# jopohl/urh

Hardware: AMD Instinct MI355X
Metric: Msamples/s IQ->bits (1 GiB complex64 2-FSK per GPU, qad materialised, compact outputs copied to the host) (higher is better)
Workload: dtype f32

## Files before the change

include/urhgpu.h:

```cpp
#ifndef URHGPU_H
#define URHGPU_H

#include <stdint.h>

#ifdef __cplusplus
extern "C" {
#endif

#define URHGPU_VERSION 100

#define URHGPU_OK 0
#define URHGPU_ERR_HIP (-1)
#define URHGPU_ERR_DTYPE (-2)
#define URHGPU_ERR_ARG (-3)
#define URHGPU_ERR_CAPACITY (-4)
#define URHGPU_ERR_UNSUPPORTED (-5)
#define URHGPU_ERR_NO_DEVICE (-6)

#define URHGPU_DT_I8 0
#define URHGPU_DT_U8 1
#define URHGPU_DT_I16 2
#define URHGPU_DT_U16 3
#define URHGPU_DT_F32 4

// ... 268 lines not shown
int urhgpu_test_hot_probe(urhgpu_ctx *ctx, const void *d_iq, int64_t n, const urhgpu_params *p, float *d_qad, int stream_kind, int event_mode,
                          int graded, int launches, int keep, void *d_chunks_out, int64_t *n_chunks_out, float *dur_ms, float *gap_ms, int bubble_us,
                          int load_kind);
int urhgpu_test_hot_stamps(int on);
int urhgpu_test_tail_skip(int mask);
int urhgpu_test_fetch_chunk_tables(urhgpu_ctx *ctx, void *host_dst, int64_t n_chunks);
int urhgpu_memcpy_to_host(urhgpu_ctx *ctx, const void *d_src, void *host_dst, int64_t bytes);
int urhgpu_memcpy_dtod(urhgpu_ctx *ctx, void *d_dst, const void *d_src, int64_t bytes);

int urhgpu_test_force_state_bytes(int on);

int urhgpu_test_force_generic_tail(int on);

int urhgpu_test_force_tiles_per_chunk(int tiles);

int64_t urhgpu_test_wide_int_launches(void);

int64_t urhgpu_test_costas_host_syncs(void);
int64_t urhgpu_test_center_host_syncs(void);
int urhgpu_test_costas_scratch(int64_t n, int loop_order, int64_t *out3);

int urhgpu_test_atan2f_dev(urhgpu_ctx *ctx, const float *d_y, const float *d_x, int64_t n, float *d_out);

int urhgpu_chunk_power_stats_dev(urhgpu_ctx *ctx, const void *d_src, int dtype, int64_t n_rows, void *d_dst, int64_t n_store, double *sum_out,
                                 double *max_out);
int urhgpu_chunk_stats_launches(urhgpu_ctx *ctx, int64_t *n_launches);

int urhgpu_magnitude_chunk_partials_dev(urhgpu_ctx *ctx, const void *d_iq, int dtype, int64_t n_local, int64_t pos_base, int64_t n_total,
                                        int64_t chunk, int64_t n_chunks, double *d_sum, double *d_max);
#define URHGPU_PW_REC_HEAD 8
// ... 63 lines not shown
```

urh_amd/_lib.py:

```python
import ctypes as C
import os
import threading

HERE = os.path.dirname(os.path.abspath(__file__))
LIB_PATH = os.path.join(HERE, "liburhgpu.so")

OK = 0
ERR_HIP, ERR_DTYPE, ERR_ARG, ERR_CAPACITY, ERR_UNSUPPORTED, ERR_NO_DEVICE = -1, -2, -3, -4, -5, -6
BLOB_LEN16 = 2
BLOB_ROW16 = 4

DT_I8, DT_U8, DT_I16, DT_U16, DT_F32 = 0, 1, 2, 3, 4
MOD_ASK, MOD_FSK, MOD_PSK, MOD_OTHER = 0, 1, 2, 3
ROW_ABSORBED = -(1 << 62)
BLOB_MAGIC = 0x55524842424C4F42
BLOB_HEADER_BYTES = 128


class UrhGpuError(RuntimeError):
    def __init__(self, status, msg):
        super().__init__(msg)
        self.status = status


# ... 161 lines not shown
    "urhgpu_modulate_gfsk": (_i, [_vp, _vp, _i64, C.c_uint32, _vp, _i, _f, _f, _f, C.c_uint32, C.c_uint32, _i, _vp, _i, _vp, _vp]),
    "urhgpu_spectrogram_dev": (_i, [_vp, _vp, _i64, _i, _i64, _i64, _vp, _vp, _vp, _vp]),
    "urhgpu_bgra_lookup_dev": (_i, [_vp, _vp, _i64, _i, _vp, _i, _f, _f, _vp]),
    "urhgpu_convert_dev": (_i, [_vp, _vp, _i, _vp, _i, _i64]),
    "urhgpu_pcm_to_iq_dev": (_i, [_vp, _vp, _i64, _i, _i, _vp]),
    "urhgpu_sub_encode_runs": (_i, [_vp, _i64, _i64, _vp, _i64, _vp]),
    "urhgpu_fft_peak_dev": (_i, [_vp, _vp, _i64, _vp]),
    "urhgpu_astype_dev": (_i, [_vp, _vp, _i, _vp, _i, _i64]),
    "urhgpu_path_minmax_dev": (_i, [_vp, _vp, _i, _i64, _i64, _i64, _vp]),
    "urhgpu_path_minmax": (_i, [_vp, _vp, _i, _i64, _i64, _i64, _i64, _vp]),
    "urhgpu_bench_copy_ceiling_dev": (_i, [_vp, _vp, _vp, _i64, _i, _i, C.POINTER(_f)]),
    "urhgpu_memcpy_to_host": (_i, [_vp, _vp, _vp, _i64]),
    "urhgpu_memcpy_dtod": (_i, [_vp, _vp, _vp, _i64]),
    "urhgpu_test_force_state_bytes": (_i, [_i]),
    "urhgpu_test_force_tiles_per_chunk": (_i, [_i]),
    "urhgpu_test_wide_int_launches": (_i64, []),
    "urhgpu_test_costas_host_syncs": (_i64, []),
    "urhgpu_test_costas_scratch": (_i, [_i64, _i, C.POINTER(_i64)]),
    "urhgpu_test_force_generic_tail": (_i, [_i]),
    "urhgpu_test_atan2f_dev": (_i, [_vp, _vp, _vp, _i64, _vp]),
    "urhgpu_chunk_power_stats_dev": (_i, [_vp, _vp, _i, _i64, _vp, _i64, C.POINTER(C.c_double), C.POINTER(C.c_double)]),
    "urhgpu_chunk_stats_launches": (_i, [_vp, C.POINTER(_i64)]),
    "urhgpu_magnitude_chunk_partials_dev": (_i, [_vp, _vp, _i, _i64, _i64, _i64, _i64, _i64, _vp, _vp]),
    "urhgpu_pairwise_partial_f32_dev": (_i, [_vp, _vp, _i64, _i64, _i64, _i, _f, _vp, _i64, C.POINTER(_i64)]),
    "urhgpu_dc_correct_dev": (_i, [_vp, _vp, _i64, _i, _vp, _vp]),
    "urhgpu_dc_correct": (_i, [_vp, _vp, _i64, _i, _vp, _vp]),
    "urhgpu_test_dc_host_syncs": (_i64, []),
    "urhgpu_test_dc_stats": (_i, [_vp, C.POINTER(_i64)]),
    "urhgpu_shard_dc_sums_dev": (_i, [_vp, _vp, _i64, _i, _vp]),
    "urhgpu_shard_dc_spec_dev": (_i, [_vp, _vp, _i64, C.POINTER(C.c_double), _vp]),
# ... 158 lines not shown
```

urh_amd/csrc/launchers.hpp:

```cpp
#pragma once
#include <atomic>
#include <hip/hip_runtime.h>
#include <stdint.h>

#include "common.hpp"
#include "runs.hpp"

namespace urh {

struct RunArgs {
    const void *in;
    float *qad;
    const void *left_halo;
    int64_t n;
    int64_t range_begin;
    int64_t range_end;
    int64_t chunk_base;
    int64_t pos_base;
    int64_t chunk_len;
    uint64_t *slab;
    int64_t slab_stride;
    ChunkInfo *chunks;
    float noise_sqrd;
    float noise_val;
// ... 7 lines not shown
    uint32_t *progress;
    int32_t n_seg;
    int32_t seg_end[kMaxSegments];
    int64_t launch_lo, launch_hi;
    int64_t graded_from, graded_len;
    int wide_int;
    int stamp_probe;
    float thr[kMaxOrder - 1];
    const float *d_thr;
    const float *d_noise;
};
extern bool g_force_state_bytes;
extern std::atomic<long long> g_wide_int_launches;
extern bool g_stamp_probe;
extern int g_tail_skip;
struct HotEvents { hipEvent_t start = nullptr, stop = nullptr; bool used = false; };
int launch_wide_probe(const void *d_iq, int dtype, int64_t n, float noise_sqrd, int32_t *h_out, hipStream_t s, const float *d_noise = nullptr);
int launch_demod_runs_iq(const RunArgs &a, int dtype, int mod, bool write_qad, hipStream_t s, HotEvents *ev = nullptr);
int launch_runs_qad(const RunArgs &a, hipStream_t s, HotEvents *ev = nullptr);
bool runs_streamable(const RunArgs &a);
int launch_afp_demod(const RunArgs &a, int dtype, int mod, int grid, hipStream_t s);
int launch_afp_seam(const RunArgs &a, int dtype, int mod, float *d_out, hipStream_t s);
void launch_test_div(uint64_t seed, int reps, unsigned long long *d_mismatches, hipStream_t s);
void launch_test_sincosf_fast(unsigned long long *d_mismatches, hipStream_t s);
void launch_test_atan2f(const float *y, const float *x, int64_t n, float *out, hipStream_t s);

struct ModMsg {
    int64_t bit_off;
    int64_t n_sym;
    int64_t sym_off;
// ... 285 lines not shown
```

urh_amd/csrc/probes.hip:

```cpp
#include "pass.hpp"

using namespace urh;

#define URH_PROBE_WPB 4

namespace urh {
bool g_tile_tail = true;
int g_force_tiles_per_chunk = 0;
}

extern "C" {

int urhgpu_test_fast_division_dev(urhgpu_ctx *ctx, uint64_t seed, int reps, uint64_t *n_mismatch) {
    if (!ctx || !n_mismatch || reps < 0) return URHGPU_ERR_ARG;
    URH_HIP(hipSetDevice(ctx->device));
    URH_HIP(hipMemsetAsync(ctx->d_counts, 0, 8, ctx->stream));
    launch_test_div(seed, reps, (unsigned long long *)ctx->d_counts, ctx->stream);
    URH_HIP(hipGetLastError());
    URH_TRY(fetch_out(ctx, ctx->h_counts, ctx->d_counts, 8));
    *n_mismatch = (uint64_t)ctx->h_counts[0];
    return URHGPU_OK;
}

int urhgpu_test_force_merge_ambiguous(int on) {
// ... 156 lines not shown
int urhgpu_test_force_generic_tail(int on) { urh::g_tile_tail = (on == 0); return URHGPU_OK; }
int64_t urhgpu_test_wide_int_launches(void) { return (int64_t)urh::g_wide_int_launches.load(); }
int64_t urhgpu_test_costas_host_syncs(void) { return (int64_t)urh::g_costas_host_syncs.load(); }
int urhgpu_test_costas_scratch(int64_t n, int loop_order, int64_t *out3) {
    if (!out3 || n < 0 || (loop_order != 2 && loop_order != 4)) return URHGPU_ERR_ARG;
    urh::costas_scratch_layout(n, loop_order == 4 ? 8 : 4, out3);
    return URHGPU_OK;
}

int urhgpu_test_force_tiles_per_chunk(int tiles) {
    if (tiles < 0 || tiles > 4) return URHGPU_ERR_ARG;
    urh::g_force_tiles_per_chunk = tiles;
    return URHGPU_OK;
}

int urhgpu_test_atan2f_dev(urhgpu_ctx *ctx, const float *d_y, const float *d_x, int64_t n, float *d_out) {
    if (!ctx) return URHGPU_ERR_ARG;
    URH_HIP(hipSetDevice(ctx->device));
    launch_test_atan2f(d_y, d_x, n, d_out, ctx->stream);
    URH_HIP(hipGetLastError());
    return URHGPU_OK;
}

}
```

urh_amd/csrc/pulse_table.hip:

```cpp
#include <hip/hip_runtime.h>

#include <algorithm>

#include "common.hpp"
#include "compact.hpp"
#include "launchers.hpp"
#include "runs.hpp"
#include "scan.hpp"

namespace urh {

#ifndef URH_RESOLVE_BLOCK
#define URH_RESOLVE_BLOCK 256
#endif
#ifndef URH_RESOLVE_ITEMS
#define URH_RESOLVE_ITEMS 4
#endif
constexpr int kResolveBlock = URH_RESOLVE_BLOCK;

__host__ __device__ static inline int64_t resolve_blocks(int64_t n_chunks) { return (n_chunks + kResolveBlock - 1) / kResolveBlock; }

size_t resolve_scratch_bytes(int64_t n_chunks) {
    return (size_t)n_chunks * (4 * 4 + 2 * 8) + (size_t)(resolve_blocks(n_chunks) + 1) * (4 + 4 + 8) + 10 * 256;
}
// ... 624 lines not shown
}
__device__ __forceinline__ ResElem res_of_chunk(int cnt, uint32_t c_first_state, uint32_t c_last_state, uint32_t c_pend_state, int64_t c_last_pos,
                                                int64_t c_pend_pos, int pend_stable) {
    const bool pend_in = pend_stable && (cnt == 0 || c_pend_state != c_last_state);
    const int k = cnt + (pend_in ? 1 : 0);
    if (k == 0) return res_identity();
    const uint32_t first_state = cnt > 0 ? c_first_state : c_pend_state;
    const int64_t last_pos = pend_in ? c_pend_pos : c_last_pos;
    const uint32_t last_state = pend_in ? c_pend_state : c_last_state;
    return res_make(first_state, k == 1 ? last_pos : -1, last_state, k - 1, k >= 2, last_pos, last_state);
}

struct TileTail {
    ResElem *ploc;
    ResElem *btot;
    VecK<4> *agg;
    VecK<4> *excl;
    int64_t *tile_off;
    int32_t *tile_cnt;
    int64_t *d_n_tiles;
    int32_t *huge_count;
    int parity;
    int want_bits;
    GranDesc *rdesc;
    unsigned long long epoch;
    int64_t *d_row_base;
    int64_t *esc;
};

__global__ __launch_bounds__(kResolveBlock) void k_resolve_one(const ResolveArgs a, const TileTail ft, const int64_t blk0, const SegGate gate) {
// ... 46 lines not shown
    if (lane == 63) s_w[wave] = incl;
    __syncthreads();
    ResElem base = res_identity(), tot = res_identity();
#pragma unroll
    for (int w = 0; w < kResolveBlock / 64; ++w) {
        if (w < wave) base = res_combine(base, s_w[w]);
        tot = res_combine(tot, s_w[w]);
    }
    ResElem ex = res_shfl_up(incl, 1);
    if (lane == 0) ex = res_identity();
    ex = res_combine(base, ex);
    if (c < a.n_chunks) ft.ploc[c] = ex;
    if (t == 0) ft.btot[blk] = tot;
}

__device__ __forceinline__ ResElem res_fold_blocks(const ResElem *btot, int64_t count, int lane, ResElem first) {
    ResElem carry = res_identity();
    for (int64_t u0 = 0; u0 < count; u0 += 64) {
        ResElem x = first;
        if (u0 > 0) { x = res_identity(); if (u0 + lane < count) x = btot[u0 + lane]; }
        x = res_wave_incl_scan(x, lane);
        carry = res_combine(carry, res_shfl(x, 63));
    }
    return carry;
}

__device__ __forceinline__ ResElem res_before_entry(const TileTail &ft, const ResElem &init, int64_t c, int64_t n_chunks, int lane) {
    const int64_t nb = (c >= n_chunks) ? resolve_blocks(n_chunks) : c / kResolveBlock;
    ResElem first = res_identity();
    if (lane < nb) first = ft.btot[lane];
    ResElem pre = res_combine(init, res_fold_blocks(ft.btot, nb, lane, first));
    if (c < n_chunks) pre = res_combine(pre, ft.ploc[c]);
    return pre;
}

struct ShardPart { ResElem tot; int32_t first_nonlead, open_chunk; };
__global__ __launch_bounds__(kResolveBlock) void k_shard_summary(const ResolveArgs a, ShardPart *part, int32_t *ticket) {
    URH_TAIL_PRIO();
    __shared__ ResElem s_w[kResolveBlock / 64];
    __shared__ int32_t s_fn[kResolveBlock / 64], s_oc[kResolveBlock / 64];
    __shared__ bool s_last;
    const int64_t c = (int64_t)blockIdx.x * kResolveBlock + threadIdx.x;
    const int t = threadIdx.x, lane = t & 63, wave = t >> 6;
    ResElem e = res_identity();
    int32_t fn = kAuxNone, oc = kAuxNone;
    if (c < a.n_chunks) {
        const ChunkInfo *ch = a.chunks + c;
        const int64_t pend_pos = ch->pend_pos, start = ch->start, len = ch->len, last_pos = ch->last_pos, own_lead = ch->lead;
// ... 125 lines not shown
#else
#define URH_EMIT_OCC
#endif
#ifdef URH_OCC_EXPAND
#define URH_EXPAND_OCC __attribute__((amdgpu_waves_per_eu(URH_OCC_EXPAND)))
#else
#define URH_EXPAND_OCC URH_TAIL_OCC
#endif
static_assert(kResolveBlock % kTailCPW == 0 && kTailCPW <= 64, "the chunks of one wavefront share their resolve workgroup");

__device__ __forceinline__ int64_t lane_bcast(int64_t v, int src) {
    const int lo = __builtin_amdgcn_readlane((int)(uint32_t)(uint64_t)v, src), hi = __builtin_amdgcn_readlane((int)(uint32_t)((uint64_t)v >> 32), src);
    return (int64_t)(((uint64_t)(uint32_t)hi << 32) | (uint32_t)lo);
}
__device__ __forceinline__ int lane_bcast(int v, int src) { return __builtin_amdgcn_readlane(v, src); }

struct EmitTileArgs {
    EmitArgs e;
    ResolveArgs r;
    TileTail ft;
    BitsParams bp;
    HugeRef *huge;
    int32_t huge_cap;
    int64_t w0, w_end;
    int final_seg;
    SegState *seg;
    int seg_k;
    int8_t *h_state;
    int32_t *h_len;
    int len16;
// ... 12 lines not shown
            const unsigned long long slot = atomicAdd((unsigned long long *)g.esc, 1ull);
            if ((int64_t)slot < g.esc_cap) g.esc[1 + slot] = (int64_t)(((uint64_t)(uint32_t)(int32_t)len << 32) | (uint64_t)(uint32_t)idx);
        }
        return;
    }
    g.h_state[idx] = (int8_t)state;
    if (!g.len16) { g.h_len[idx] = (int32_t)len; return; }
    const bool fits = len >= 0 && len < 0xFFFF;
    ((uint16_t *)g.h_len)[idx] = fits ? (uint16_t)len : (uint16_t)0xFFFF;
    if (!fits) {
        const unsigned long long slot = atomicAdd((unsigned long long *)g.esc, 1ull);
        if ((int64_t)slot < g.esc_cap) g.esc[1 + slot] = (int64_t)(((uint64_t)(uint32_t)(int32_t)len << 32) | (uint64_t)(uint32_t)idx);
    }
}

template <int TC>
__global__ __launch_bounds__(64 * kEmitWaves) URH_EMIT_OCC void k_emit_rows_tiles(const EmitTileArgs g) {
    URH_TAIL_PRIO();
    const EmitArgs &a = g.e;
    const ResolveArgs &r = g.r;
    const int lane = threadIdx.x & 63;
    const int64_t w = g.w0 + (int64_t)blockIdx.x * kEmitWaves + __builtin_amdgcn_readfirstlane((int)(threadIdx.x >> 6));
    const int64_t n_cw = g.w_end;
    if (w > n_cw) return;
    const bool totals = (w == n_cw);
    const bool table = (r.n_local != r.n_chunks);
    const int64_t lc0 = a.chunk_first, lc1 = a.chunk_first + r.n_local;
    const int64_t c0 = totals ? (g.final_seg ? r.n_chunks : n_cw * kTailCPW) : w * kTailCPW;
    const int64_t n_before = (totals && g.final_seg) ? resolve_blocks(r.n_chunks) : c0 / kResolveBlock;
    const uint32_t init_state = a.chunks[0].init_state;
    ResElem first = res_identity();
    if (lane < n_before) first = g.ft.btot[lane];
    const int n_mine = totals ? 0 : (int)((r.n_chunks - c0 < kTailCPW) ? r.n_chunks - c0 : kTailCPW);
    ResElem pl_l = res_identity();
    int cnt_l = 0, fl_l = 0, pp_l = 0;
    int64_t pend_pos_l = -1, last_pos_l = 0;
    if (lane < n_mine) {
        pl_l = g.ft.ploc[c0 + lane];
        const ChunkInfo *ch = a.chunks + c0 + lane;
        cnt_l = ch->cnt; pend_pos_l = ch->pend_pos;
        if (table) last_pos_l = ch->last_pos;
        fl_l = (int)((uint32_t)ch->first_state | ((uint32_t)ch->last_state << 16));
        pp_l = (int)((uint32_t)ch->pend_state | ((uint32_t)(ch->pend_stable ? 1 : 0) << 16));
    }
    uint64_t rec = 0;
    if (n_mine > 0 && c0 >= lc0 && c0 < lc1 && lane < a.slab_stride)
        rec = (a.slab + (c0 - lc0) * a.slab_stride)[lane];
    const ResElem init = res_make(init_state, -1, init_state, 0, false, -1, 0);
    const ResElem base = res_combine(init, res_fold_blocks(g.ft.btot, n_before, lane, first));
    int64_t row_base = 0;
    if (table) row_base = res_before_entry(g.ft, init, lc0, r.n_chunks, lane).cnt;
    if (totals) {
        const ResElem pre = base;
        if (!g.final_seg) {
            if (lane == 0) g.seg->rows_at[g.seg_k] = (r.rows != nullptr && pre.cnt > r.cap_rows) ? r.cap_rows : pre.cnt;
            return;
        }
        const int64_t c = chunk_tiles(r.n_chunks, TC);
        int64_t row_end = pre.cnt;
        if (table && lc1 < r.n_chunks) row_end = res_before_entry(g.ft, init, lc1, r.n_chunks, lane).cnt;
        if (lane == 0) {
            const int64_t P = pre.cnt;
            *r.d_n_acc = P;
            int64_t n_rows = row_end - row_base;
            int64_t o = n_rows;
            VecK<4> v; v.zero();
            int32_t tcnt = 0;
            if (P < r.n_total && r.write_last_row) {
                o = P - row_base;
                n_rows = o + 1;
                tcnt = 1;
                const int64_t fpos = pre.la_valid() ? pre.la_pos : -1;
                const uint32_t fstate = pre.la_valid() ? pre.la_state() : init_state;
                const int64_t len = (P == 0) ? (r.n_total - r.tol) : (r.n_total - 1 - fpos - r.tol);
                if (r.rows != nullptr && o < r.cap_rows) {
                    r.rows[2 * o] = (int64_t)fstate - 1; r.rows[2 * o + 1] = len;
                    if (g.h_state) ship_row(g, o, (int64_t)fstate - 1, len);
                }
                if (g.ft.want_bits) {
                    v = row_value((int64_t)fstate - 1, len, P == 0, g.bp);
                    if (v.v[0] > kHugeBits) {
                        const int slot = atomicAdd(g.ft.huge_count + g.ft.parity, 1);
                        if (slot < g.huge_cap) { g.huge[slot].tile = c; g.huge[slot].row = o; }
                    }
                }
            }
            *r.d_n_rows_needed = n_rows;
            *r.d_n_rows = (r.rows != nullptr && n_rows > r.cap_rows) ? r.cap_rows : n_rows;
            if (g.ft.d_row_base) *g.ft.d_row_base = row_base;
            g.ft.agg[c] = v; g.ft.tile_off[c] = o; g.ft.tile_cnt[c] = tcnt;
        }
        return;
    }
    int64_t acc_bits = 0;
    uint64_t acc_ld = 0;
    int64_t my_last_pos = 0;
    int64_t t_samples = 0, t_off = 0, t_total = 0;
    for (int jc = 0; jc < n_mine; ++jc) {
        const int64_t c = c0 + jc;
        const bool local = (TC > 1) || (c >= lc0 && c < lc1);
        const uint64_t *slab = a.slab + (c - lc0) * a.slab_stride;
        uint64_t rec_next = 0;
        if (jc + 1 < n_mine && c + 1 >= lc0 && c + 1 < lc1 && lane < a.slab_stride) rec_next = (a.slab + (c + 1 - lc0) * a.slab_stride)[lane];
        ResElem pl;
        pl.cnt = lane_bcast(pl_l.cnt, jc); pl.first_pos = lane_bcast(pl_l.first_pos, jc); pl.la_pos = lane_bcast(pl_l.la_pos, jc);
        pl.meta = (uint64_t)lane_bcast((int64_t)pl_l.meta, jc);
        const int cnt = lane_bcast(cnt_l, jc);
        const uint32_t fl = (uint32_t)lane_bcast(fl_l, jc), pp = (uint32_t)lane_bcast(pp_l, jc);
        const int64_t pend_pos = lane_bcast(pend_pos_l, jc);
        const uint32_t c_first = fl & 0xFFFFu, c_last = fl >> 16, c_pend = pp & 0xFFFFu;
        const int pend_stable = (int)(pp >> 16);
        const ResElem pre = res_combine(base, pl);
        const uint32_t prev_state = pre.last_state();
        const int first_acc = (cnt > 0) && (c_first != prev_state);
        const uint32_t before_pend = (cnt > 0) ? c_last : prev_state;
        const int pend_acc = pend_stable && (c_pend != before_pend);
        const int skip = (cnt > 0 && !first_acc) ? 1 : 0;
        const int64_t from_slab = (cnt > 0) ? cnt - skip : 0;
        const int64_t total = from_slab + pend_acc;
        const int64_t out_off = pre.cnt;
        const int64_t prev_pos = pre.la_valid() ? pre.la_pos : -1;
        const uint32_t prev_st = pre.la_valid() ? pre.la_state() : init_state;
        if (!local) {
            VecK<4> acc; acc.zero();
            if (g.ft.want_bits && total > 0) acc.v[2] = (pend_acc ? pend_pos : lane_bcast(last_pos_l, jc)) - prev_pos;
            if (lane == 0) { g.ft.agg[c] = acc; g.ft.tile_off[c] = 0; g.ft.tile_cnt[c] = 0; }
            rec = rec_next;
            continue;
        }
        if (jc % TC == 0) { acc_bits = 0; acc_ld = 0; t_samples = 0; t_total = 0; t_off = out_off - row_base; }
        const bool in_regs = cnt <= 64;
        const uint64_t rec_j = skip ? (uint64_t)__shfl_down((long long)rec, 1) : rec;
        const uint64_t rec_p = (uint64_t)__shfl_up((long long)rec_j, 1);
        for (int64_t j = lane; j < total; j += 64) {
            int64_t pos, ppos; uint32_t pst;
            if (in_regs && j < 64) {
                pos = (j < from_slab) ? rec_pos(rec_j) : pend_pos;
                if (j == 0) { ppos = prev_pos; pst = prev_st; }
                else { ppos = rec_pos(rec_p); pst = rec_state(rec_p); }
            } else {
                pos = (j < from_slab) ? rec_pos(slab[j + skip]) : pend_pos;
                if (j == 0) { ppos = prev_pos; pst = prev_st; }
                else { const uint64_t rr = slab[j - 1 + skip]; ppos = rec_pos(rr); pst = rec_state(rr); }
            }
            my_last_pos = pos;
            const int64_t gi = out_off + j;
            const int64_t len = (gi == 0) ? pos + 1 : pos - ppos;
            const int64_t state = (int64_t)pst - 1;
            if (gi - row_base < a.cap_rows) {
                if (a.rows) *(longlong2 *)(a.rows + 2 * (gi - row_base)) = longlong2{(long long)state, (long long)len};
                if (g.h_state) ship_row(g, gi - row_base, state, len);
            }
            if (g.ft.want_bits) {
                const VecK<4> v = row_value(state, len, gi == 0, g.bp);
                acc_bits += v.v[0];
                acc_ld += (uint64_t)v.v[1] | ((uint64_t)v.v[3] << 32);
                if (v.v[0] > kHugeBits) {
                    const int slot = atomicAdd(g.ft.huge_count + g.ft.parity, 1);
                    if (slot < g.huge_cap) { g.huge[slot].tile = c / TC; g.huge[slot].row = gi - row_base; }
                }
            }
        }
        if (g.ft.want_bits && total > 0) t_samples += lane_bcast(my_last_pos, (int)((total - 1) & 63)) - prev_pos;
        t_total += total;
        if (jc % TC == TC - 1 || jc == n_mine - 1) {
            VecK<4> acc; acc.zero();
            if (g.ft.want_bits && t_total > 0) {
#pragma unroll
                for (int o = 32; o > 0; o >>= 1) { acc_bits += __shfl_xor(acc_bits, o); acc_ld += (uint64_t)__shfl_xor((long long)acc_ld, o); }
                acc.v[0] = acc_bits; acc.v[1] = (int64_t)(acc_ld & 0xFFFFFFFFull); acc.v[3] = (int64_t)(acc_ld >> 32);
                acc.v[2] = t_samples;
            }
            if (lane == 0) { g.ft.agg[c / TC] = acc; g.ft.tile_off[c / TC] = t_off; g.ft.tile_cnt[c / TC] = (int32_t)t_total; }
        }
        rec = rec_next;
    }
}

struct TileScanArgs {
    const int64_t *rows;
    const int64_t *d_n_rows;
    const VecK<4> *agg;
    const int64_t *tile_off;
    const int32_t *tile_cnt;
    VecK<4> *excl;
    GroupInfo *groups;
    int64_t cap_groups;
    int64_t *d_n_groups;
// ... 498 lines not shown
    return launch_bits_finish(rows, d_n_rows, cap_rows, bp, o, scratch, ss, s);
}


int g_tail_skip = 0;
namespace {
constexpr int kTileHugeCap = 8192;
struct TileCarve { TileTail ft; HugeRef *huge; };
TileCarve carve_tile(const TileTailMem &m) {
    TileCarve tc;
    char *p = (char *)m.mem;
    auto take = [&](size_t bytes) { char *r = p; p += (bytes + 255) & ~size_t(255); return r; };
    const int64_t nt = m.n_chunks + 1;
    tc.ft.ploc = (ResElem *)take((size_t)m.n_chunks * sizeof(ResElem));
    tc.ft.btot = (ResElem *)take((size_t)(resolve_blocks(m.n_chunks) + 1) * sizeof(ResElem));
    tc.ft.agg = (VecK<4> *)take((size_t)nt * sizeof(VecK<4>));
    tc.ft.excl = (VecK<4> *)take((size_t)nt * sizeof(VecK<4>));
    tc.ft.tile_off = (int64_t *)take((size_t)nt * 8);
    tc.ft.tile_cnt = (int32_t *)take((size_t)nt * 4);
    tc.ft.d_n_tiles = (int64_t *)take(64);
    tc.huge = (HugeRef *)take((size_t)kTileHugeCap * sizeof(HugeRef));
    tc.ft.huge_count = m.huge_count;
    tc.ft.parity = m.parity;
    tc.ft.want_bits = 0;
    tc.ft.rdesc = (GranDesc *)m.rdesc;
    tc.ft.epoch = m.epoch;
    tc.ft.d_row_base = m.d_row_base;
    tc.ft.esc = nullptr;
    return tc;
}
// ... 3 lines not shown

int64_t tile_desc_cap(int64_t cap_rows, int64_t n_chunks) { return std::max<int64_t>(cap_rows, 8 * (n_chunks + 2) + kScanTile); }

static inline int64_t tile_scan_blocks_tc(int64_t c0, int64_t c1, int final, int tc) {
    const int64_t t1 = final ? chunk_tiles(c1, tc) + 1 : c1 / tc;
    return (t1 - c0 / tc + kScanBlock - 1) / kScanBlock;
}
int64_t tile_scan_blocks(int64_t c0, int64_t c1, int final) { return tile_scan_blocks_tc(c0, c1, final, kTileChunks); }

size_t tile_rdesc_bytes(int64_t n_chunks) {
    return (size_t)(resolve_blocks(n_chunks) + 2 + (n_chunks + 1 + kScanBlock - 1) / kScanBlock + kMaxSegments + 2) * sizeof(GranDesc);
}

size_t tile_tail_bytes(int64_t n_chunks) {
    const int64_t nt = n_chunks + 1;
    return (size_t)n_chunks * sizeof(ResElem) + (size_t)(resolve_blocks(n_chunks) + 1) * sizeof(ResElem) + (size_t)nt * (2 * sizeof(VecK<4>) + 12) +
           64 + (size_t)kTileHugeCap * sizeof(HugeRef) + 10 * 256;
}

int launch_tile_rows(const ResolveArgs &r, const EmitArgs &e, const TileTailMem &m, const BitsParams *bp, hipStream_t s) {
    if (r.n_chunks <= 0 || r.local_pass || r.chunk_first != e.chunk_first || r.chunk_first < 0 || r.chunk_first + r.n_local > r.n_chunks ||
        m.n_chunks != r.n_chunks || e.is_ask)
        return URHGPU_ERR_ARG;
    if ((r.n_local != r.n_chunks) != (m.d_row_base != nullptr)) return URHGPU_ERR_ARG;
    TileCarve tc = carve_tile(m);
    EmitTileArgs g;
    g.e = e; g.r = r; g.ft = tc.ft; g.huge = tc.huge; g.huge_cap = kTileHugeCap;
    memset(&g.bp, 0, sizeof(g.bp));
    if (bp) { g.bp = *bp; g.ft.want_bits = 1; }
    const unsigned gb = (unsigned)resolve_blocks(r.n_chunks);
    g.w0 = 0; g.w_end = tail_waves(r.n_chunks); g.final_seg = 1; g.seg = nullptr; g.seg_k = 0; g.h_state = nullptr; g.h_len = nullptr; g.len16 = 0; g.esc = nullptr; g.esc_cap = 0; g.ft.esc = nullptr;
    SegGate no_gate;
    memset(&no_gate, 0, sizeof(no_gate));
    if (!(g_tail_skip & 1)) hipLaunchKernelGGL(k_resolve_one, dim3(gb), dim3(kResolveBlock), 0, s, r, g.ft, (int64_t)0, no_gate);
    const dim3 grid((unsigned)((tail_waves(r.n_chunks) + 1 + kEmitWaves - 1) / kEmitWaves));
    if (!(g_tail_skip & 2)) {
        if (tile_chunks_of(m) == 1) hipLaunchKernelGGL(k_emit_rows_tiles<1>, grid, dim3(64 * kEmitWaves), 0, s, g);
        else hipLaunchKernelGGL(k_emit_rows_tiles<kTileChunks>, grid, dim3(64 * kEmitWaves), 0, s, g);
    }
    return URHGPU_OK;
}

namespace {
__global__ void k_tile_flags(const int64_t *d_n_rows, const GroupInfo *groups, const int64_t *d_n_groups, int64_t *d_flags) {
    const int64_t n = *d_n_rows, ng = *d_n_groups;
    const int64_t n_l = (n > 0 && ng > 0) ? ng - 1 : 0;
    d_flags[0] = n_l > 0;
    d_flags[1] = (n > 0) && groups[0].data_end > 0;
    d_flags[2] = (n > 0) && (groups[n_l].data_end - (n_l ? groups[n_l - 1].data_end : 0) > 0);
}
}

int launch_tile_bits_prepare(const TileTailMem &m, const int64_t *rows, const int64_t *d_n_rows, int64_t cap_rows, const BitsParams &bp,
                             void *scratch, int64_t *d_flags, const ScanState &ss, hipStream_t s) {
// ... 224 lines not shown
    const TileCarve tc = carve_tile(m);
    EmitTileArgs g;
    g.e = e; g.r = r; g.ft = tc.ft; g.huge = tc.huge; g.huge_cap = kTileHugeCap;
    g.bp = bp; g.ft.want_bits = 1;
    g.w0 = sg.c0 / kTailCPW; g.w_end = sg.final ? tail_waves(r.n_chunks) : sg.c1 / kTailCPW; g.final_seg = sg.final; g.seg = state; g.seg_k = sg.index;
    g.h_state = sg.h_state; g.h_len = sg.h_len;
    g.len16 = (sg.len16 && sg.esc && sg.h_len) ? sg.len16 : 0; g.esc = g.len16 ? sg.esc : nullptr; g.esc_cap = sg.esc_cap;
    g.ft.esc = (g.len16 && sg.index == 0) ? sg.esc : nullptr;
    if (g_tail_skip & 64) { g.h_state = nullptr; g.h_len = nullptr; }
    if (g_tail_skip & 128) g.e.rows = nullptr;
    TileTail ft_resolve = g.ft;
    if (sg.index != 0) ft_resolve.want_bits = 0;
    SegGate gate = sg.gate;
    gate.fused = (sg.fuse_gate && gate.progress && !gate.init && resolve_blocks(sg.c1 - sg.c0) == 1) ? 1 : 0;
    if (!gate.fused && gate.progress) hipLaunchKernelGGL(k_seg_gate, dim3(1), dim3(64), 0, s, gate);
    if (!(g_tail_skip & 1)) hipLaunchKernelGGL(k_resolve_one, dim3((unsigned)resolve_blocks(sg.c1 - sg.c0)), dim3(kResolveBlock), 0, s, r, ft_resolve, sg.c0 / kResolveBlock, gate);
    if (!(g_tail_skip & 2)) hipLaunchKernelGGL(k_emit_rows_tiles<kTileChunks>, dim3((unsigned)((g.w_end - g.w0 + 1 + kEmitWaves - 1) / kEmitWaves)), dim3(64 * kEmitWaves), 0, s, g);
    return URHGPU_OK;
}

int launch_bits_segment(const TileTailMem &m, const BitsParams &bp, const BitsOut &o, void *scratch, const ScanState &ss, int64_t *rows,
                        int64_t cap_rows, const BitsSegment &sg, const SegPackDst *dst, hipStream_t s) {
    if (m.n_chunks <= 0 || m.d_row_base != nullptr || !sg.state || sg.rows_index < 0 || sg.rows_index >= kMaxSegments) return URHGPU_ERR_ARG;
    if (sg.c0 < 0 || sg.c0 % kSegAlign || sg.c1 <= sg.c0 || sg.c1 > m.n_chunks || (sg.final ? sg.c1 != m.n_chunks : (sg.c1 % kSegAlign != 0 || sg.c1 >= m.n_chunks)))
        return URHGPU_ERR_ARG;
    if (cap_rows <= 0) cap_rows = 1;
    const int64_t cap_desc = tile_desc_cap(cap_rows, m.n_chunks);
    if (ss.desc_bytes < bits_desc_bytes(cap_desc)) return URHGPU_ERR_ARG;
    const TileCarve tc = carve_tile(m);
    const BitsScratch b = carve_bits(scratch, cap_rows);
    SegState *st = sg.state;
    const int64_t *d_n_rows = &st->rows_at[sg.rows_index];
// ... 106 lines not shown
```

Baseline: 489,300.

## Precompute resolve-block prefixes once and add 32-bit row emit path

```diff
diff --git a/include/urhgpu.h b/include/urhgpu.h
--- a/include/urhgpu.h
+++ b/include/urhgpu.h
@@ -306,6 +306,10 @@
 
 int urhgpu_test_force_tiles_per_chunk(int tiles);
 
+int urhgpu_test_force_rows64(int on);
+int64_t urhgpu_test_rows32_launches(void);
+int urhgpu_test_rows32_ok(int64_t n_total, int64_t cap_rows, int64_t sps, int64_t bps, int64_t pause_threshold);
+
 int64_t urhgpu_test_wide_int_launches(void);
 
 int64_t urhgpu_test_costas_host_syncs(void);
diff --git a/urh_amd/_lib.py b/urh_amd/_lib.py
--- a/urh_amd/_lib.py
+++ b/urh_amd/_lib.py
@@ -199,6 +199,9 @@
     "urhgpu_memcpy_dtod": (_i, [_vp, _vp, _vp, _i64]),
     "urhgpu_test_force_state_bytes": (_i, [_i]),
     "urhgpu_test_force_tiles_per_chunk": (_i, [_i]),
+    "urhgpu_test_force_rows64": (_i, [_i]),
+    "urhgpu_test_rows32_launches": (_i64, []),
+    "urhgpu_test_rows32_ok": (_i, [_i64, _i64, _i64, _i64, _i64]),
     "urhgpu_test_wide_int_launches": (_i64, []),
     "urhgpu_test_costas_host_syncs": (_i64, []),
     "urhgpu_test_costas_scratch": (_i, [_i64, _i, C.POINTER(_i64)]),
diff --git a/urh_amd/csrc/launchers.hpp b/urh_amd/csrc/launchers.hpp
--- a/urh_amd/csrc/launchers.hpp
+++ b/urh_amd/csrc/launchers.hpp
@@ -45,6 +45,9 @@
 extern std::atomic<long long> g_wide_int_launches;
 extern bool g_stamp_probe;
 extern int g_tail_skip;
+extern bool g_force_rows64;
+extern std::atomic<long long> g_rows32_launches;
+bool rows32_ok(int64_t n_total, int64_t cap_rows, int64_t sps, int64_t bps, int64_t pause_threshold);
 struct HotEvents { hipEvent_t start = nullptr, stop = nullptr; bool used = false; };
 int launch_wide_probe(const void *d_iq, int dtype, int64_t n, float noise_sqrd, int32_t *h_out, hipStream_t s, const float *d_noise = nullptr);
 int launch_demod_runs_iq(const RunArgs &a, int dtype, int mod, bool write_qad, hipStream_t s, HotEvents *ev = nullptr);
diff --git a/urh_amd/csrc/probes.hip b/urh_amd/csrc/probes.hip
--- a/urh_amd/csrc/probes.hip
+++ b/urh_amd/csrc/probes.hip
@@ -194,6 +194,12 @@
     return URHGPU_OK;
 }
 
+int urhgpu_test_force_rows64(int on) { urh::g_force_rows64 = (on != 0); return URHGPU_OK; }
+int64_t urhgpu_test_rows32_launches(void) { return (int64_t)urh::g_rows32_launches.load(); }
+int urhgpu_test_rows32_ok(int64_t n_total, int64_t cap_rows, int64_t sps, int64_t bps, int64_t pause_threshold) {
+    return urh::rows32_ok(n_total, cap_rows, sps, bps, pause_threshold) ? 1 : 0;
+}
+
 int urhgpu_test_atan2f_dev(urhgpu_ctx *ctx, const float *d_y, const float *d_x, int64_t n, float *d_out) {
     if (!ctx) return URHGPU_ERR_ARG;
     URH_HIP(hipSetDevice(ctx->device));
diff --git a/urh_amd/csrc/pulse_table.hip b/urh_amd/csrc/pulse_table.hip
--- a/urh_amd/csrc/pulse_table.hip
+++ b/urh_amd/csrc/pulse_table.hip
@@ -1,6 +1,8 @@
 #include <hip/hip_runtime.h>
 
 #include <algorithm>
+#include <atomic>
+#include <type_traits>
 
 #include "common.hpp"
 #include "compact.hpp"
@@ -662,6 +664,7 @@
 struct TileTail {
     ResElem *ploc;
     ResElem *btot;
+    ResElem *bbase;
     VecK<4> *agg;
     VecK<4> *excl;
     int64_t *tile_off;
@@ -738,24 +741,29 @@
     if (t == 0) ft.btot[blk] = tot;
 }
 
-__device__ __forceinline__ ResElem res_fold_blocks(const ResElem *btot, int64_t count, int lane, ResElem first) {
-    ResElem carry = res_identity();
-    for (int64_t u0 = 0; u0 < count; u0 += 64) {
-        ResElem x = first;
-        if (u0 > 0) { x = res_identity(); if (u0 + lane < count) x = btot[u0 + lane]; }
+__global__ __launch_bounds__(64) void k_block_prefix(const ChunkInfo *chunks, const TileTail ft, const int64_t blk0, const int64_t nblk) {
+    URH_TAIL_PRIO();
+    const int lane = threadIdx.x;
+    ResElem x = res_identity();
+    if (lane < nblk) x = ft.btot[blk0 + lane];
+    const uint32_t init_state = chunks[0].init_state;
+    const ResElem prev = ft.bbase[blk0];
+    const ResElem init = res_make(init_state, -1, init_state, 0, false, -1, 0);
+    ResElem carry;
+    carry.cnt = blk0 ? prev.cnt : init.cnt; carry.first_pos = blk0 ? prev.first_pos : init.first_pos;
+    carry.la_pos = blk0 ? prev.la_pos : init.la_pos; carry.meta = blk0 ? prev.meta : init.meta;
+    if (blk0 == 0 && lane == 0) ft.bbase[0] = carry;
+    for (int64_t u0 = 0; u0 < nblk; u0 += 64) {
+        if (u0 > 0) { x = res_identity(); if (u0 + lane < nblk) x = ft.btot[blk0 + u0 + lane]; }
         x = res_wave_incl_scan(x, lane);
+        if (u0 + lane < nblk) ft.bbase[blk0 + u0 + lane + 1] = res_combine(carry, x);
         carry = res_combine(carry, res_shfl(x, 63));
     }
-    return carry;
-}
-
-__device__ __forceinline__ ResElem res_before_entry(const TileTail &ft, const ResElem &init, int64_t c, int64_t n_chunks, int lane) {
-    const int64_t nb = (c >= n_chunks) ? resolve_blocks(n_chunks) : c / kResolveBlock;
-    ResElem first = res_identity();
-    if (lane < nb) first = ft.btot[lane];
-    ResElem pre = res_combine(init, res_fold_blocks(ft.btot, nb, lane, first));
-    if (c < n_chunks) pre = res_combine(pre, ft.ploc[c]);
-    return pre;
+}
+
+__device__ __forceinline__ ResElem res_before_entry(const TileTail &ft, int64_t c, int64_t n_chunks) {
+    if (c >= n_chunks) return ft.bbase[resolve_blocks(n_chunks)];
+    return res_combine(ft.bbase[c / kResolveBlock], ft.ploc[c]);
 }
 
 struct ShardPart { ResElem tot; int32_t first_nonlead, open_chunk; };
@@ -911,6 +919,10 @@
     return (int64_t)(((uint64_t)(uint32_t)hi << 32) | (uint32_t)lo);
 }
 __device__ __forceinline__ int lane_bcast(int v, int src) { return __builtin_amdgcn_readlane(v, src); }
+__device__ __forceinline__ int64_t lane_bcast_first(int64_t v) {
+    const int lo = __builtin_amdgcn_readfirstlane((int)(uint32_t)(uint64_t)v), hi = __builtin_amdgcn_readfirstlane((int)(uint32_t)((uint64_t)v >> 32));
+    return (int64_t)(((uint64_t)(uint32_t)hi << 32) | (uint32_t)lo);
+}
 
 struct EmitTileArgs {
     EmitArgs e;
@@ -953,8 +965,86 @@
     }
 }
 
-template <int TC>
+
+__device__ __forceinline__ ResElem res_uniform(const ResElem &x) {
+    ResElem r;
+    r.cnt = lane_bcast_first(x.cnt); r.first_pos = lane_bcast_first(x.first_pos); r.la_pos = lane_bcast_first(x.la_pos);
+    r.meta = (uint64_t)lane_bcast_first((int64_t)x.meta);
+    return r;
+}
+
+__device__ __forceinline__ void row_value32(int32_t state, int32_t len, bool global_row0, uint32_t sps, uint32_t bps, uint32_t pause_threshold,
+                                            uint32_t &kb, uint32_t &lp, uint32_t &dr) {
+    kb = 0; lp = 0; dr = 0;
+    if (global_row0 && state == -1) return;
+    const uint32_t q = (uint32_t)len / sps, rem = (uint32_t)len - q * sps;
+    const uint32_t ns = q + ((rem > sps - rem) ? 1u : 0u);
+    if (state == -1) {
+        if (ns <= pause_threshold || pause_threshold == 0) kb = ns * bps;
+        else lp = 1;
+    } else {
+        kb = ns * bps;
+        dr = (ns > 0) ? 1u : 0u;
+    }
+}
+
+template <int TC, bool TABLE>
+__device__ __forceinline__ void emit_totals(const EmitTileArgs &g, int lane) {
+    const ResolveArgs &r = g.r;
+    const int64_t n_cw = g.w_end;
+    const int64_t nb = g.final_seg ? resolve_blocks(r.n_chunks) : n_cw * kTailCPW / kResolveBlock;
+    const uint32_t init_state = g.e.chunks[0].init_state;
+    const ResElem pre = res_uniform(g.ft.bbase[nb]);
+    if (!g.final_seg) {
+        if (lane == 0) g.seg->rows_at[g.seg_k] = (r.rows != nullptr && pre.cnt > r.cap_rows) ? r.cap_rows : pre.cnt;
+        return;
+    }
+    const int64_t lc0 = g.e.chunk_first, lc1 = g.e.chunk_first + r.n_local;
+    int64_t row_base = 0;
+    int64_t row_end = pre.cnt;
+    if (TABLE) {
+        row_base = res_before_entry(g.ft, lc0, r.n_chunks).cnt;
+        if (lc1 < r.n_chunks) row_end = res_before_entry(g.ft, lc1, r.n_chunks).cnt;
+    }
+    const int64_t c = chunk_tiles(r.n_chunks, TC);
+    if (lane == 0) {
+        const int64_t P = pre.cnt;
+        *r.d_n_acc = P;
+        int64_t n_rows = row_end - row_base;
+        int64_t o = n_rows;
+        VecK<4> v; v.zero();
+        int32_t tcnt = 0;
+        if (P < r.n_total && r.write_last_row) {
+            o = P - row_base;
+            n_rows = o + 1;
+            tcnt = 1;
+            const int64_t fpos = pre.la_valid() ? pre.la_pos : -1;
+            const uint32_t fstate = pre.la_valid() ? pre.la_state() : init_state;
+            const int64_t len = (P == 0) ? (r.n_total - r.tol) : (r.n_total - 1 - fpos - r.tol);
+            if (r.rows != nullptr && o < r.cap_rows) {
+                r.rows[2 * o] = (int64_t)fstate - 1; r.rows[2 * o + 1] = len;
+                if (g.h_state) ship_row(g, o, (int64_t)fstate - 1, len);
+            }
+            if (g.ft.want_bits) {
+                v = row_value((int64_t)fstate - 1, len, P == 0, g.bp);
+                if (v.v[0] > kHugeBits) {
+                    const int slot = atomicAdd(g.ft.huge_count + g.ft.parity, 1);
+                    if (slot < g.huge_cap) { g.huge[slot].tile = c; g.huge[slot].row = o; }
+                }
+            }
+        }
+        *r.d_n_rows_needed = n_rows;
+        *r.d_n_rows = (r.rows != nullptr && n_rows > r.cap_rows) ? r.cap_rows : n_rows;
+        if (g.ft.d_row_base) *g.ft.d_row_base = row_base;
+        g.ft.agg[c] = v; g.ft.tile_off[c] = o; g.ft.tile_cnt[c] = tcnt;
+    }
+}
+
+template <int TC, bool TABLE, bool R32>
 __global__ __launch_bounds__(64 * kEmitWaves) URH_EMIT_OCC void k_emit_rows_tiles(const EmitTileArgs g) {
+    static_assert(!TABLE || (TC == 1 && !R32), "table passes of sharded captures: one chunk per tile, 64-bit rows");
+    using P = typename std::conditional<R32, int32_t, int64_t>::type;
+    using U = typename std::conditional<R32, uint32_t, int64_t>::type;
     URH_TAIL_PRIO();
     const EmitArgs &a = g.e;
     const ResolveArgs &r = g.r;
@@ -962,91 +1052,49 @@
     const int64_t w = g.w0 + (int64_t)blockIdx.x * kEmitWaves + __builtin_amdgcn_readfirstlane((int)(threadIdx.x >> 6));
     const int64_t n_cw = g.w_end;
     if (w > n_cw) return;
-    const bool totals = (w == n_cw);
-    const bool table = (r.n_local != r.n_chunks);
+    if (w == n_cw) { emit_totals<TC, TABLE>(g, lane); return; }
     const int64_t lc0 = a.chunk_first, lc1 = a.chunk_first + r.n_local;
-    const int64_t c0 = totals ? (g.final_seg ? r.n_chunks : n_cw * kTailCPW) : w * kTailCPW;
-    const int64_t n_before = (totals && g.final_seg) ? resolve_blocks(r.n_chunks) : c0 / kResolveBlock;
+    const int64_t c0 = w * kTailCPW;
     const uint32_t init_state = a.chunks[0].init_state;
-    ResElem first = res_identity();
-    if (lane < n_before) first = g.ft.btot[lane];
-    const int n_mine = totals ? 0 : (int)((r.n_chunks - c0 < kTailCPW) ? r.n_chunks - c0 : kTailCPW);
-    ResElem pl_l = res_identity();
+    const ResElem base_v = g.ft.bbase[c0 / kResolveBlock];
+    const int n_mine = (int)((r.n_chunks - c0 < kTailCPW) ? r.n_chunks - c0 : kTailCPW);
+    P pl_cnt = 0, pl_first = -1, pl_la = -1;
+    uint64_t pl_meta = 0;
     int cnt_l = 0, fl_l = 0, pp_l = 0;
-    int64_t pend_pos_l = -1, last_pos_l = 0;
+    P pend_pos_l = -1, last_pos_l = 0;
     if (lane < n_mine) {
-        pl_l = g.ft.ploc[c0 + lane];
+        const ResElem pl = g.ft.ploc[c0 + lane];
+        pl_cnt = (P)pl.cnt; pl_first = (P)pl.first_pos; pl_la = (P)pl.la_pos; pl_meta = pl.meta;
         const ChunkInfo *ch = a.chunks + c0 + lane;
-        cnt_l = ch->cnt; pend_pos_l = ch->pend_pos;
-        if (table) last_pos_l = ch->last_pos;
+        cnt_l = ch->cnt; pend_pos_l = (P)ch->pend_pos;
+        if (TABLE) last_pos_l = (P)ch->last_pos;
         fl_l = (int)((uint32_t)ch->first_state | ((uint32_t)ch->last_state << 16));
         pp_l = (int)((uint32_t)ch->pend_state | ((uint32_t)(ch->pend_stable ? 1 : 0) << 16));
     }
     uint64_t rec = 0;
-    if (n_mine > 0 && c0 >= lc0 && c0 < lc1 && lane < a.slab_stride)
+    if (n_mine > 0 && (!TABLE || (c0 >= lc0 && c0 < lc1)) && lane < a.slab_stride)
         rec = (a.slab + (c0 - lc0) * a.slab_stride)[lane];
-    const ResElem init = res_make(init_state, -1, init_state, 0, false, -1, 0);
-    const ResElem base = res_combine(init, res_fold_blocks(g.ft.btot, n_before, lane, first));
-    int64_t row_base = 0;
-    if (table) row_base = res_before_entry(g.ft, init, lc0, r.n_chunks, lane).cnt;
-    if (totals) {
-        const ResElem pre = base;
-        if (!g.final_seg) {
-            if (lane == 0) g.seg->rows_at[g.seg_k] = (r.rows != nullptr && pre.cnt > r.cap_rows) ? r.cap_rows : pre.cnt;
-            return;
-        }
-        const int64_t c = chunk_tiles(r.n_chunks, TC);
-        int64_t row_end = pre.cnt;
-        if (table && lc1 < r.n_chunks) row_end = res_before_entry(g.ft, init, lc1, r.n_chunks, lane).cnt;
-        if (lane == 0) {
-            const int64_t P = pre.cnt;
-            *r.d_n_acc = P;
-            int64_t n_rows = row_end - row_base;
-            int64_t o = n_rows;
-            VecK<4> v; v.zero();
-            int32_t tcnt = 0;
-            if (P < r.n_total && r.write_last_row) {
-                o = P - row_base;
-                n_rows = o + 1;
-                tcnt = 1;
-                const int64_t fpos = pre.la_valid() ? pre.la_pos : -1;
-                const uint32_t fstate = pre.la_valid() ? pre.la_state() : init_state;
-                const int64_t len = (P == 0) ? (r.n_total - r.tol) : (r.n_total - 1 - fpos - r.tol);
-                if (r.rows != nullptr && o < r.cap_rows) {
-                    r.rows[2 * o] = (int64_t)fstate - 1; r.rows[2 * o + 1] = len;
-                    if (g.h_state) ship_row(g, o, (int64_t)fstate - 1, len);
-                }
-                if (g.ft.want_bits) {
-                    v = row_value((int64_t)fstate - 1, len, P == 0, g.bp);
-                    if (v.v[0] > kHugeBits) {
-                        const int slot = atomicAdd(g.ft.huge_count + g.ft.parity, 1);
-                        if (slot < g.huge_cap) { g.huge[slot].tile = c; g.huge[slot].row = o; }
-                    }
-                }
-            }
-            *r.d_n_rows_needed = n_rows;
-            *r.d_n_rows = (r.rows != nullptr && n_rows > r.cap_rows) ? r.cap_rows : n_rows;
-            if (g.ft.d_row_base) *g.ft.d_row_base = row_base;
-            g.ft.agg[c] = v; g.ft.tile_off[c] = o; g.ft.tile_cnt[c] = tcnt;
-        }
-        return;
-    }
-    int64_t acc_bits = 0;
+    P row_base = 0;
+    if (TABLE) row_base = (P)res_before_entry(g.ft, lc0, r.n_chunks).cnt;
+    const ResElem base = res_uniform(base_v);
+    const P cap = R32 ? (P)(a.cap_rows < INT32_MAX ? a.cap_rows : INT32_MAX) : (P)a.cap_rows;
+    const uint32_t sps32 = (uint32_t)g.bp.sps, bps32 = (uint32_t)g.bp.bps, pt32 = (uint32_t)g.bp.pause_threshold;
+    U acc_bits = 0;
     uint64_t acc_ld = 0;
-    int64_t my_last_pos = 0;
-    int64_t t_samples = 0, t_off = 0, t_total = 0;
+    P my_last_pos = 0;
+    P t_samples = 0, t_off = 0, t_total = 0;
     for (int jc = 0; jc < n_mine; ++jc) {
         const int64_t c = c0 + jc;
-        const bool local = (TC > 1) || (c >= lc0 && c < lc1);
+        const bool local = !TABLE || (c >= lc0 && c < lc1);
         const uint64_t *slab = a.slab + (c - lc0) * a.slab_stride;
         uint64_t rec_next = 0;
-        if (jc + 1 < n_mine && c + 1 >= lc0 && c + 1 < lc1 && lane < a.slab_stride) rec_next = (a.slab + (c + 1 - lc0) * a.slab_stride)[lane];
+        if (jc + 1 < n_mine && (!TABLE || (c + 1 >= lc0 && c + 1 < lc1)) && lane < a.slab_stride) rec_next = (a.slab + (c + 1 - lc0) * a.slab_stride)[lane];
         ResElem pl;
-        pl.cnt = lane_bcast(pl_l.cnt, jc); pl.first_pos = lane_bcast(pl_l.first_pos, jc); pl.la_pos = lane_bcast(pl_l.la_pos, jc);
-        pl.meta = (uint64_t)lane_bcast((int64_t)pl_l.meta, jc);
+        pl.cnt = lane_bcast(pl_cnt, jc); pl.first_pos = lane_bcast(pl_first, jc); pl.la_pos = lane_bcast(pl_la, jc);
+        pl.meta = (uint64_t)lane_bcast((int64_t)pl_meta, jc);
         const int cnt = lane_bcast(cnt_l, jc);
         const uint32_t fl = (uint32_t)lane_bcast(fl_l, jc), pp = (uint32_t)lane_bcast(pp_l, jc);
-        const int64_t pend_pos = lane_bcast(pend_pos_l, jc);
+        const P pend_pos = lane_bcast(pend_pos_l, jc);
         const uint32_t c_first = fl & 0xFFFFu, c_last = fl >> 16, c_pend = pp & 0xFFFFu;
         const int pend_stable = (int)(pp >> 16);
         const ResElem pre = res_combine(base, pl);
@@ -1055,12 +1103,12 @@
         const uint32_t before_pend = (cnt > 0) ? c_last : prev_state;
         const int pend_acc = pend_stable && (c_pend != before_pend);
         const int skip = (cnt > 0 && !first_acc) ? 1 : 0;
-        const int64_t from_slab = (cnt > 0) ? cnt - skip : 0;
-        const int64_t total = from_slab + pend_acc;
-        const int64_t out_off = pre.cnt;
-        const int64_t prev_pos = pre.la_valid() ? pre.la_pos : -1;
+        const P from_slab = (cnt > 0) ? cnt - skip : 0;
+        const P total = from_slab + pend_acc;
+        const P out_off = (P)pre.cnt;
+        const P prev_pos = pre.la_valid() ? (P)pre.la_pos : (P)-1;
         const uint32_t prev_st = pre.la_valid() ? pre.la_state() : init_state;
-        if (!local) {
+        if (TABLE && !local) {
             VecK<4> acc; acc.zero();
             if (g.ft.want_bits && total > 0) acc.v[2] = (pend_acc ? pend_pos : lane_bcast(last_pos_l, jc)) - prev_pos;
             if (lane == 0) { g.ft.agg[c] = acc; g.ft.tile_off[c] = 0; g.ft.tile_cnt[c] = 0; }
@@ -1071,32 +1119,43 @@
         const bool in_regs = cnt <= 64;
         const uint64_t rec_j = skip ? (uint64_t)__shfl_down((long long)rec, 1) : rec;
         const uint64_t rec_p = (uint64_t)__shfl_up((long long)rec_j, 1);
-        for (int64_t j = lane; j < total; j += 64) {
-            int64_t pos, ppos; uint32_t pst;
+        for (P j = lane; j < total; j += 64) {
+            P pos, ppos; uint32_t pst;
             if (in_regs && j < 64) {
-                pos = (j < from_slab) ? rec_pos(rec_j) : pend_pos;
+                pos = (j < from_slab) ? (P)rec_pos(rec_j) : pend_pos;
                 if (j == 0) { ppos = prev_pos; pst = prev_st; }
-                else { ppos = rec_pos(rec_p); pst = rec_state(rec_p); }
+                else { ppos = (P)rec_pos(rec_p); pst = rec_state(rec_p); }
             } else {
-                pos = (j < from_slab) ? rec_pos(slab[j + skip]) : pend_pos;
+                pos = (j < from_slab) ? (P)rec_pos(slab[j + skip]) : pend_pos;
                 if (j == 0) { ppos = prev_pos; pst = prev_st; }
-                else { const uint64_t rr = slab[j - 1 + skip]; ppos = rec_pos(rr); pst = rec_state(rr); }
+                else { const uint64_t rr = slab[j - 1 + skip]; ppos = (P)rec_pos(rr); pst = rec_state(rr); }
             }
             my_last_pos = pos;
-            const int64_t gi = out_off + j;
-            const int64_t len = (gi == 0) ? pos + 1 : pos - ppos;
-            const int64_t state = (int64_t)pst - 1;
-            if (gi - row_base < a.cap_rows) {
-                if (a.rows) *(longlong2 *)(a.rows + 2 * (gi - row_base)) = longlong2{(long long)state, (long long)len};
-                if (g.h_state) ship_row(g, gi - row_base, state, len);
+            const P gi = out_off + j;
+            const P ri = gi - row_base;
+            const P len = (gi == 0) ? pos + 1 : pos - ppos;
+            const P state = (P)pst - 1;
+            if (ri < cap) {
+                if (a.rows) *(longlong2 *)(a.rows + 2 * (int64_t)ri) = longlong2{(long long)state, (long long)len};
+                if (g.h_state) ship_row(g, (int64_t)ri, (int64_t)state, (int64_t)len);
             }
             if (g.ft.want_bits) {
-                const VecK<4> v = row_value(state, len, gi == 0, g.bp);
-                acc_bits += v.v[0];
-                acc_ld += (uint64_t)v.v[1] | ((uint64_t)v.v[3] << 32);
-                if (v.v[0] > kHugeBits) {
+                bool huge;
+                if constexpr (R32) {
+                    uint32_t kb, lp, dr;
+                    row_value32(state, len, gi == 0, sps32, bps32, pt32, kb, lp, dr);
+                    acc_bits += kb;
+                    acc_ld += (uint64_t)lp | ((uint64_t)dr << 32);
+                    huge = kb > (uint32_t)kHugeBits;
+                } else {
+                    const VecK<4> v = row_value(state, len, gi == 0, g.bp);
+                    acc_bits += v.v[0];
+                    acc_ld += (uint64_t)v.v[1] | ((uint64_t)v.v[3] << 32);
+                    huge = v.v[0] > kHugeBits;
+                }
+                if (huge) {
                     const int slot = atomicAdd(g.ft.huge_count + g.ft.parity, 1);
-                    if (slot < g.huge_cap) { g.huge[slot].tile = c / TC; g.huge[slot].row = gi - row_base; }
+                    if (slot < g.huge_cap) { g.huge[slot].tile = c / TC; g.huge[slot].row = (int64_t)ri; }
                 }
             }
         }
@@ -1105,12 +1164,13 @@
         if (jc % TC == TC - 1 || jc == n_mine - 1) {
             VecK<4> acc; acc.zero();
             if (g.ft.want_bits && t_total > 0) {
+                int64_t sum_bits = (int64_t)acc_bits;
 #pragma unroll
-                for (int o = 32; o > 0; o >>= 1) { acc_bits += __shfl_xor(acc_bits, o); acc_ld += (uint64_t)__shfl_xor((long long)acc_ld, o); }
-                acc.v[0] = acc_bits; acc.v[1] = (int64_t)(acc_ld & 0xFFFFFFFFull); acc.v[3] = (int64_t)(acc_ld >> 32);
-                acc.v[2] = t_samples;
-            }
-            if (lane == 0) { g.ft.agg[c / TC] = acc; g.ft.tile_off[c / TC] = t_off; g.ft.tile_cnt[c / TC] = (int32_t)t_total; }
+                for (int o = 32; o > 0; o >>= 1) { sum_bits += __shfl_xor(sum_bits, o); acc_ld += (uint64_t)__shfl_xor((long long)acc_ld, o); }
+                acc.v[0] = sum_bits; acc.v[1] = (int64_t)(acc_ld & 0xFFFFFFFFull); acc.v[3] = (int64_t)(acc_ld >> 32);
+                acc.v[2] = (int64_t)t_samples;
+            }
+            if (lane == 0) { g.ft.agg[c / TC] = acc; g.ft.tile_off[c / TC] = (int64_t)t_off; g.ft.tile_cnt[c / TC] = (int32_t)t_total; }
         }
         rec = rec_next;
     }
@@ -1639,6 +1699,7 @@
     const int64_t nt = m.n_chunks + 1;
     tc.ft.ploc = (ResElem *)take((size_t)m.n_chunks * sizeof(ResElem));
     tc.ft.btot = (ResElem *)take((size_t)(resolve_blocks(m.n_chunks) + 1) * sizeof(ResElem));
+    tc.ft.bbase = (ResElem *)take((size_t)(resolve_blocks(m.n_chunks) + 1) * sizeof(ResElem));
     tc.ft.agg = (VecK<4> *)take((size_t)nt * sizeof(VecK<4>));
     tc.ft.excl = (VecK<4> *)take((size_t)nt * sizeof(VecK<4>));
     tc.ft.tile_off = (int64_t *)take((size_t)nt * 8);
@@ -1672,8 +1733,33 @@
 
 size_t tile_tail_bytes(int64_t n_chunks) {
     const int64_t nt = n_chunks + 1;
-    return (size_t)n_chunks * sizeof(ResElem) + (size_t)(resolve_blocks(n_chunks) + 1) * sizeof(ResElem) + (size_t)nt * (2 * sizeof(VecK<4>) + 12) +
-           64 + (size_t)kTileHugeCap * sizeof(HugeRef) + 10 * 256;
+    return (size_t)n_chunks * sizeof(ResElem) + 2 * (size_t)(resolve_blocks(n_chunks) + 1) * sizeof(ResElem) + (size_t)nt * (2 * sizeof(VecK<4>) + 12) +
+           64 + (size_t)kTileHugeCap * sizeof(HugeRef) + 11 * 256;
+}
+
+bool g_force_rows64 = false;
+std::atomic<long long> g_rows32_launches{0};
+
+bool rows32_ok(int64_t n_total, int64_t cap_rows, int64_t sps, int64_t bps, int64_t pause_threshold) {
+    if (n_total < 0 || n_total > INT32_MAX) return false;
+    if (bps <= 0) return true;
+    if (sps < 1 || sps > (int64_t)UINT32_MAX || pause_threshold < 0 || pause_threshold > (int64_t)UINT32_MAX || bps > INT32_MAX) return false;
+    const int64_t rows = std::max<int64_t>(std::max<int64_t>(cap_rows, 0), n_total / 64 + 1);
+    return n_total / sps + rows + 1 <= (int64_t)INT32_MAX / bps;
+}
+
+namespace {
+void launch_emit_rows_tiles(const EmitTileArgs &g, bool table, dim3 grid, hipStream_t s) {
+    const dim3 block(64 * kEmitWaves);
+    if (table) { hipLaunchKernelGGL((k_emit_rows_tiles<1, true, false>), grid, block, 0, s, g); return; }
+    const bool r32 = !g_force_rows64 && rows32_ok(g.r.n_total, g.e.cap_rows, g.bp.sps, g.ft.want_bits ? g.bp.bps : 0, g.bp.pause_threshold);
+    if (r32) {
+        g_rows32_launches.fetch_add(1, std::memory_order_relaxed);
+        hipLaunchKernelGGL((k_emit_rows_tiles<kTileChunks, false, true>), grid, block, 0, s, g);
+    } else {
+        hipLaunchKernelGGL((k_emit_rows_tiles<kTileChunks, false, false>), grid, block, 0, s, g);
+    }
+}
 }
 
 int launch_tile_rows(const ResolveArgs &r, const EmitArgs &e, const TileTailMem &m, const BitsParams *bp, hipStream_t s) {
@@ -1690,12 +1776,12 @@
     g.w0 = 0; g.w_end = tail_waves(r.n_chunks); g.final_seg = 1; g.seg = nullptr; g.seg_k = 0; g.h_state = nullptr; g.h_len = nullptr; g.len16 = 0; g.esc = nullptr; g.esc_cap = 0; g.ft.esc = nullptr;
     SegGate no_gate;
     memset(&no_gate, 0, sizeof(no_gate));
-    if (!(g_tail_skip & 1)) hipLaunchKernelGGL(k_resolve_one, dim3(gb), dim3(kResolveBlock), 0, s, r, g.ft, (int64_t)0, no_gate);
+    if (!(g_tail_skip & 1)) {
+        hipLaunchKernelGGL(k_resolve_one, dim3(gb), dim3(kResolveBlock), 0, s, r, g.ft, (int64_t)0, no_gate);
+        hipLaunchKernelGGL(k_block_prefix, dim3(1), dim3(64), 0, s, (const ChunkInfo *)r.chunks, g.ft, (int64_t)0, (int64_t)gb);
+    }
     const dim3 grid((unsigned)((tail_waves(r.n_chunks) + 1 + kEmitWaves - 1) / kEmitWaves));
-    if (!(g_tail_skip & 2)) {
-        if (tile_chunks_of(m) == 1) hipLaunchKernelGGL(k_emit_rows_tiles<1>, grid, dim3(64 * kEmitWaves), 0, s, g);
-        else hipLaunchKernelGGL(k_emit_rows_tiles<kTileChunks>, grid, dim3(64 * kEmitWaves), 0, s, g);
-    }
+    if (!(g_tail_skip & 2)) launch_emit_rows_tiles(g, m.d_row_base != nullptr, grid, s);
     return URHGPU_OK;
 }
 
@@ -1950,8 +2036,12 @@
     SegGate gate = sg.gate;
     gate.fused = (sg.fuse_gate && gate.progress && !gate.init && resolve_blocks(sg.c1 - sg.c0) == 1) ? 1 : 0;
     if (!gate.fused && gate.progress) hipLaunchKernelGGL(k_seg_gate, dim3(1), dim3(64), 0, s, gate);
-    if (!(g_tail_skip & 1)) hipLaunchKernelGGL(k_resolve_one, dim3((unsigned)resolve_blocks(sg.c1 - sg.c0)), dim3(kResolveBlock), 0, s, r, ft_resolve, sg.c0 / kResolveBlock, gate);
-    if (!(g_tail_skip & 2)) hipLaunchKernelGGL(k_emit_rows_tiles<kTileChunks>, dim3((unsigned)((g.w_end - g.w0 + 1 + kEmitWaves - 1) / kEmitWaves)), dim3(64 * kEmitWaves), 0, s, g);
+    if (!(g_tail_skip & 1)) {
+        const int64_t nblk = resolve_blocks(sg.c1 - sg.c0);
+        hipLaunchKernelGGL(k_resolve_one, dim3((unsigned)nblk), dim3(kResolveBlock), 0, s, r, ft_resolve, sg.c0 / kResolveBlock, gate);
+        hipLaunchKernelGGL(k_block_prefix, dim3(1), dim3(64), 0, s, (const ChunkInfo *)r.chunks, g.ft, sg.c0 / kResolveBlock, nblk);
+    }
+    if (!(g_tail_skip & 2)) launch_emit_rows_tiles(g, false, dim3((unsigned)((g.w_end - g.w0 + 1 + kEmitWaves - 1) / kEmitWaves)), s);
     return URHGPU_OK;
 }
 
```

Measured after the change: 487,100. No clear change (-0.5%).
